# songrise/AvatarCraft

Hardware: AMD Instinct MI355X
Metric: rays/sec, 4096-ray batch, 256x256 render (64+64 samples/ray) (higher is better)
Workload: dtype f32

## Files before the change

### avatarcraft_amd/csrc/nsr_device.hpp

```cpp
#pragma once
#include "ac_common.hpp"
#include "ac_devmath.hpp"
#include "ac_sp_table.hpp"
#include "ac_sh16.hpp"

using namespace acdev;

typedef float f32x4 __attribute__((ext_vector_type(4)));

namespace {

#ifndef AC_WPB
#define AC_WPB 8
#endif
constexpr int WAVES_PER_BLOCK = AC_WPB;
constexpr int BLOCK = WAVES_PER_BLOCK * 64;
constexpr int MAXT = 128;
constexpr int SEG_STATE = MAXT + 16 + 64;
#ifndef AC_ENC_ROUND
#define AC_ENC_ROUND 2
#endif

constexpr int OFF_W1F = 0;
constexpr int OFF_W2F = OFF_W1F + 4 * 9 * 64;
// ... 7 lines not shown
constexpr int SPQ_FLOATS = 129 * 4;
constexpr int OFF_SPQ = OFF_LIN + 80;
constexpr int OFF_WAVE = OFF_SPQ + SPQ_FLOATS;
constexpr int FE_SLAB = 6 * 8 * 64;
constexpr int OFF_W1H = OFF_WAVE;
constexpr int OFF_W1L = OFF_W1H + 4 * 64 * 4;
constexpr int OFF_W1C = OFF_W1L + 4 * 64 * 4;
constexpr int CF_FRAGS = 14, CF_FRAG = 64 * 4;
constexpr int OFF_CFH = OFF_C1F;
constexpr int OFF_CFL = OFF_C1F + CF_FRAGS * CF_FRAG;
constexpr int OFF_C3L = OFF_W1C + 3 * 64;
static_assert(OFF_CFL + 12 * CF_FRAG == OFF_B1, "the bf16 colour fragments fill the fp32 colour region exactly");
constexpr int OFF_RWAVE = OFF_C3L + 2 * CF_FRAG;
constexpr int CF_OVERLAY = OFF_B1 - OFF_C1F;
constexpr int UPS_FLOATS = MAXT + 2 * MAXT + MAXT + 32;
constexpr int SLAB_ACC = MAXT + (FE_SLAB > UPS_FLOATS ? FE_SLAB : UPS_FLOATS);
constexpr int SLAB_SHB = SLAB_ACC + 16;
constexpr int WAVE_SLAB = SLAB_SHB + 80;
constexpr int LDS_FLOATS = OFF_RWAVE + WAVES_PER_BLOCK * WAVE_SLAB;
static_assert(LDS_FLOATS * 4 <= 160 * 1024, "LDS budget: one workgroup per CU");
static_assert(OFF_WAVE % 4 == 0 && OFF_RWAVE % 4 == 0 && WAVE_SLAB % 4 == 0, "16-byte aligned slabs");

#ifdef AC_PROFILE
#define AC_T0() unsigned long long t_prof_ = __builtin_amdgcn_s_memtime(); const unsigned long long ray_r0_ = __builtin_amdgcn_s_memrealtime()
#define AC_TICK(SLOT) { const unsigned long long t2_ = __builtin_amdgcn_s_memtime(); prof_acc[SLOT] += t2_ - t_prof_; t_prof_ = t2_; }
#else
#define AC_T0()
#define AC_TICK(SLOT)
#endif

struct LevelRec { float scale; uint32_t my, mz, offset, mask, hashed, wsize, pad; };

struct RenderArgs {
    const float *table;
    uint32_t table_bytes;
    const float *W1, *b1, *W2, *b2, *Wc1, *Wc2, *Wc3;
    const float *Wsh;
    const float *prepared;
    const float *rays_o, *rays_d, *bg, *noise, *lin_z, *lin_u;
    ac_render_out out;
    LevelRec lvl[16];
    int n_rays, T0, nup;
    int jmode[4];
    int jfine[4];
    float bound, two_bound, inv_s, car, one_m_car, eps;
    float inv_tb;
    const float *inv_s_dev;
    int fast;
    int skip_masked;
    int opacity_only;
    int perturb;
    unsigned long long *prof;
    const float *near_m, *far_m;
    const float *ext_pts;
    const uint8_t *mask;
    uint32_t *ray_counter;
    uint32_t *seg_flags;
    float *seg_state;
    uint64_t seg_cb;
    int seg_n;
    int pair_n;
    uint32_t *done_counter;
    uint32_t *handoff_timeouts;
    float *eik_red;
    uint32_t gen;
    int ex_from;
    int ex_rows;
    const uint8_t *ray_dead;
    float *zbuf;
    float *mid_pts;
};

enum { MODE_FULL = 0, MODE_UPSAMPLE = 2, MODE_FINAL = 3 };

__device__ __forceinline__ void cube_near_far(float ox, float oy, float oz, float dx, float dy, float dz, float bound, float &near, float &far)
{
    const float ex = dx + 1e-15f, ey = dy + 1e-15f, ez = dz + 1e-15f;
    const float ax = (-bound - ox) / ex, bx = (bound - ox) / ex;
    const float ay = (-bound - oy) / ey, by = (bound - oy) / ey;
    const float az = (-bound - oz) / ez, bz = (bound - oz) / ez;
    const float lx = ax < bx ? ax : bx, hx = ax > bx ? ax : bx;
    const float ly = ay < by ? ay : by, hy = ay > by ? ay : by;
    const float lz = az < bz ? az : bz, hz = az > bz ? az : bz;
    near = lx; if (ly > near) near = ly; if (lz > near) near = lz;
    far = hx; if (hy < far) far = hy; if (hz < far) far = hz;
    if (near < 0.05f) near = 0.05f;
}
__device__ __forceinline__ bool is_inf(float v) { return __builtin_fabsf(v) == __builtin_inff(); }

__device__ __forceinline__ void wave_sync()
{
    __builtin_amdgcn_fence(__ATOMIC_ACQ_REL, "wavefront");
    __builtin_amdgcn_wave_barrier();
}

template <int OFF> __device__ __forceinline__ float dpp_shr(float ident, float v)
{
    return __builtin_bit_cast(float, __builtin_amdgcn_update_dpp(__builtin_bit_cast(int, ident), __builtin_bit_cast(int, v),
                                                                  0x110 + OFF, 0xf, 0xf, false));
}
template <bool MUL> __device__ __forceinline__ float row_scan(float v)
{
    const float id = MUL ? 1.0f : 0.0f;
    float s;
    s = dpp_shr<1>(id, v); v = MUL ? s * v : s + v;
    s = dpp_shr<2>(id, v); v = MUL ? s * v : s + v;
    s = dpp_shr<4>(id, v); v = MUL ? s * v : s + v;
    s = dpp_shr<8>(id, v); v = MUL ? s * v : s + v;
    return v;
}
__device__ __forceinline__ float lane_bcast(float v, int lane)
{
    return __builtin_bit_cast(float, __builtin_amdgcn_readlane(__builtin_bit_cast(int, v), lane));
}
__device__ __forceinline__ float sel4(int g, float a, float b, float c, float d)
{
    return g == 0 ? a : (g == 1 ? b : (g == 2 ? c : d));
}

__device__ __forceinline__ void fill_lds_sdf(float *lds, const RenderArgs &a)
{
    for (int e = threadIdx.x; e < 4 * 9 * 64; e += blockDim.x) {
        int l = e & 63, fs = e >> 6, t = fs / 9, s = fs % 9;
        int u = 16 * t + (l & 15), g = l >> 4;
        int col = (s == 0) ? (g < 3 ? g : -1) : 3 + 2 * (4 * ((s - 1) >> 1) + g) + ((s - 1) & 1);
        lds[OFF_W1F + e] = col < 0 ? 0.0f : a.W1[u * 35 + col];
    }
    for (int e = threadIdx.x; e < 16 * 64; e += blockDim.x) {
        int l = e & 63, kk = e >> 6, t = kk >> 2, r = kk & 3;
        lds[OFF_W2F + e] = a.W2[(l & 15) * 64 + 16 * t + 4 * (l >> 4) + r];
    }
    for (int e = threadIdx.x; e < 64; e += blockDim.x) lds[OFF_B1 + e] = a.b1[e];
    for (int e = threadIdx.x; e < 16; e += blockDim.x) lds[OFF_B2 + e] = a.b2[e];
    {
        uint32_t *lw = reinterpret_cast<uint32_t *>(lds) + OFF_LVL;
#pragma unroll
        for (int l = 0; l < 16; ++l) {
            if (threadIdx.x == (unsigned)l) {
                lw[8 * l + 0] = __float_as_uint(a.lvl[l].scale); lw[8 * l + 1] = a.lvl[l].my;
                lw[8 * l + 2] = a.lvl[l].mz; lw[8 * l + 3] = a.lvl[l].offset;
                lw[8 * l + 4] = a.lvl[l].mask; lw[8 * l + 5] = a.lvl[l].hashed;
                lw[8 * l + 6] = a.lvl[l].wsize; lw[8 * l + 7] = 0u;
            }
        }
    }
    for (int e = threadIdx.x; e < 64; e += blockDim.x) lds[OFF_LIN + e] = e < a.T0 ? a.lin_z[e] : 0.0f;
    for (int e = threadIdx.x; e < 16; e += blockDim.x) lds[OFF_LIN + 64 + e] = a.lin_u ? a.lin_u[e] : 0.0f;
    for (int e = threadIdx.x; e < SPQ_FLOATS; e += blockDim.x) lds[OFF_SPQ + e] = AC_SP_G[e >> 2][e & 3];
}

__device__ __forceinline__ void fill_lds_color(float *lds, const RenderArgs &a)
{
    for (int e = threadIdx.x; e < 4 * 6 * 64; e += blockDim.x) {
        int l = e & 63, fs = e >> 6, t = fs / 6, s = fs % 6;
        int u = 16 * t + (l & 15), g = l >> 4;
        float v;
        if (s < 4) { int o = 4 * g + s; v = (o == 0) ? 0.0f : a.Wc1[u * 21 + 6 + (o - 1)]; }
        else if (s == 4) v = g < 3 ? a.Wc1[u * 21 + g] : 0.0f;
        else v = g < 3 ? a.Wc1[u * 21 + 3 + g] : 0.0f;
        lds[OFF_C1F + e] = v;
    }
    for (int e = threadIdx.x; e < 4 * 16 * 64; e += blockDim.x) {
        int l = e & 63, fs = e >> 6, to = fs >> 4, kk = fs & 15, t = kk >> 2, r = kk & 3;
        lds[OFF_C2F + e] = a.Wc2[(16 * to + (l & 15)) * 64 + 16 * t + 4 * (l >> 4) + r];
    }
    for (int e = threadIdx.x; e < 16 * 64; e += blockDim.x) {
        int l = e & 63, kk = e >> 6, t = kk >> 2, r = kk & 3, o = l & 15;
        lds[OFF_C3F + e] = o < 3 ? a.Wc3[o * 64 + 16 * t + 4 * (l >> 4) + r] : 0.0f;
    }
}

__device__ __forceinline__ void fill_lds(float *lds, const RenderArgs &a)
{
    fill_lds_sdf(lds, a);
    fill_lds_color(lds, a);
}

__device__ __forceinline__ uint32_t bf16_rne_bits(float f)
{
    const uint32_t u = __float_as_uint(f);
    return (u + 0x7fffu + ((u >> 16) & 1u)) >> 16;
}
template <int W1H = OFF_W1H, int W1L = OFF_W1L, int W1C = OFF_W1C>
__device__ __forceinline__ void fill_lds_fast(float *lds, const RenderArgs &a)
{
    uint32_t *lw = reinterpret_cast<uint32_t *>(lds);
    for (int e = threadIdx.x; e < 4 * 64 * 4; e += blockDim.x) {
        const int q = e & 3, l = (e >> 2) & 63, t = e >> 8;
        const int u = 16 * t + (l & 15), kk = l >> 4;
        uint32_t hi2 = 0, lo2 = 0;
#pragma unroll
        for (int h = 0; h < 2; ++h) {
            const int i = 2 * q + h;
            const float w = a.W1[u * 35 + 3 + 2 * (4 * (i >> 1) + kk) + (i & 1)];
            const uint32_t hb = bf16_rne_bits(w);
            const uint32_t lb = bf16_rne_bits(w - __uint_as_float(hb << 16));
            hi2 |= hb << (16 * h); lo2 |= lb << (16 * h);
        }
        lw[W1H + e] = hi2; lw[W1L + e] = lo2;
    }
    for (int e = threadIdx.x; e < 3 * 64; e += blockDim.x) lds[W1C + e] = a.W1[(e & 63) * 35 + (e >> 6)];
}

__device__ __forceinline__ float color_fast_weight(const RenderArgs &a, int f, int l, int i)
{
    const int m = l & 15, g = l >> 4;
    if (f < 4) {
        const int u = 16 * f + m;
        if (i < 4) { const int o = 4 * g + i; return o == 0 ? 0.0f : a.Wc1[u * 21 + 5 + o]; }
        if (i < 7 && g < 2) return a.Wc1[u * 21 + 3 * g + (i - 4)];
        return 0.0f;
    }
    const int s = (f - 4) & 1, unit = 16 * (2 * s + (i >> 2)) + 4 * g + (i & 3);
    if (f < 12) return a.Wc2[(16 * ((f - 4) >> 1) + m) * 64 + unit];
    return m < 3 ? a.Wc3[m * 64 + unit] : 0.0f;
}
template <bool OVERLAY, bool TAIL>
__device__ __forceinline__ void fill_lds_color_fast(float *lds, const RenderArgs &a)
{
    uint32_t *lw = reinterpret_cast<uint32_t *>(lds);
    for (int e = threadIdx.x; e < CF_FRAGS * CF_FRAG; e += blockDim.x) {
        const int q = e & 3, l = (e >> 2) & 63, f = e >> 8;
        if (!(f < 12 ? OVERLAY : (OVERLAY || TAIL))) continue;
        uint32_t hi2 = 0, lo2 = 0;
#pragma unroll
        for (int h = 0; h < 2; ++h) {
            const float w = color_fast_weight(a, f, l, 2 * q + h);
            const uint32_t hb = bf16_rne_bits(w);
            const uint32_t lb = bf16_rne_bits(w - __uint_as_float(hb << 16));
            hi2 |= hb << (16 * h); lo2 |= lb << (16 * h);
        }
        if (OVERLAY) lw[OFF_CFH + e] = hi2;
        if (f < 12) { if (OVERLAY) lw[OFF_CFL + e] = lo2; }
        else if (TAIL) lw[OFF_C3L + (e - 12 * CF_FRAG)] = lo2;
    }
}

typedef __amdgpu_buffer_rsrc_t rsrc_t;
typedef uint32_t u32x2 __attribute__((ext_vector_type(2)));
typedef uint32_t u32q __attribute__((ext_vector_type(4)));
__device__ __forceinline__ void interp8(const u32x2 (&v)[8], float qx, float qy, float qz, bool oob, float &f0, float &f1)
{
    const float wx0 = 1.0f - qx, wy0 = 1.0f - qy, wz0 = 1.0f - qz;
    const float w00 = wx0 * wy0, w10 = qx * wy0, w01 = wx0 * qy, w11 = qx * qy;
    float a0 = 0.0f, a1 = 0.0f;
#pragma unroll
    for (int c = 0; c < 8; ++c) {
        const float wxy = (c & 2) ? ((c & 1) ? w11 : w01) : ((c & 1) ? w10 : w00);
        const float w = wxy * ((c & 4) ? qz : wz0);
        a0 = fma_(w, __uint_as_float(v[c].x), a0);
        a1 = fma_(w, __uint_as_float(v[c].y), a1);
    }
    f0 = oob ? 0.0f : a0;
    f1 = oob ? 0.0f : a1;
}
template <int ROUND>
__device__ __forceinline__ void encode4(const float *__restrict__ lds, rsrc_t table, int g, const int (&jmode)[4],
                                        float px, float py, float pz, float bound, float two_bound, float (&f)[4][2], float inv_tb = 0.0f)
{
    float ux, uy, uz;
    if (inv_tb != 0.0f) { ux = unit_div(px + bound, two_bound, inv_tb); uy = unit_div(py + bound, two_bound, inv_tb); uz = unit_div(pz + bound, two_bound, inv_tb); }
    else { ux = (px + bound) / two_bound; uy = (py + bound) / two_bound; uz = (pz + bound) / two_bound; }
    const bool oob = (ux < 0.0f) | (ux > 1.0f) | (uy < 0.0f) | (uy > 1.0f) | (uz < 0.0f) | (uz > 1.0f);
#pragma unroll
    for (int j0 = 0; j0 < 4; j0 += ROUND) {
        float q[ROUND][3];
        u32x2 v[ROUND][8];
#pragma unroll
        for (int jj = 0; jj < ROUND; ++jj) {
            const int j = j0 + jj;
            const uint4 r0 = *reinterpret_cast<const uint4 *>(lds + OFF_LVL + (4 * j + g) * 8);
            const uint4 r1 = *reinterpret_cast<const uint4 *>(lds + OFF_LVL + (4 * j + g) * 8 + 4);
            const float scale = __uint_as_float(r0.x);
            const uint32_t my = r0.y, mz = r0.z, offset = r0.w, mask = r1.x, hashed = r1.y;
            float qx = fma_(ux, scale, 0.5f), qy = fma_(uy, scale, 0.5f), qz = fma_(uz, scale, 0.5f);
            const uint32_t gx = (uint32_t)__builtin_floorf(qx), gy = (uint32_t)__builtin_floorf(qy), gz = (uint32_t)__builtin_floorf(qz);
            q[jj][0] = qx - (float)gx; q[jj][1] = qy - (float)gy; q[jj][2] = qz - (float)gz;
            const uint32_t ax0 = gx, ax1 = gx + 1u, ay0 = gy * my, ay1 = ay0 + my, az0 = gz * mz, az1 = az0 + mz;
            const int mode = jmode[j];
            uint32_t idx[8];
            if (mode == 0) {
#pragma unroll
                for (int c = 0; c < 8; ++c) idx[c] = ((c & 1) ? ax1 : ax0) + ((c & 2) ? ay1 : ay0) + ((c & 4) ? az1 : az0);
            } else if (mode == 1) {
#pragma unroll
                for (int c = 0; c < 8; ++c) idx[c] = (((c & 1) ? ax1 : ax0) ^ ((c & 2) ? ay1 : ay0) ^ ((c & 4) ? az1 : az0)) & mask;
            } else {
#pragma unroll
                for (int c = 0; c < 8; ++c) {
                    const uint32_t tx = (c & 1) ? ax1 : ax0, ty = (c & 2) ? ay1 : ay0, tz = (c & 4) ? az1 : az0;
                    idx[c] = (hashed ? (tx ^ ty ^ tz) : (tx + ty + tz)) & mask;
                }
            }
#pragma unroll
            for (int c = 0; c < 8; ++c) v[jj][c] = __builtin_amdgcn_raw_buffer_load_b64(table, (offset + idx[c]) * 8u, 0, 0);
        }
#pragma unroll
        for (int jj = 0; jj < ROUND; ++jj)
            interp8(v[jj], q[jj][0], q[jj][1], q[jj][2], oob, f[j0 + jj][0], f[j0 + jj][1]);
        __builtin_amdgcn_sched_barrier(0);
    }
}

struct FieldCtx { rsrc_t table; int jmode[4]; int jfine[4]; float bound, two_bound, inv_tb; };
__device__ __forceinline__ rsrc_t table_of(const FieldCtx &fc) { return fc.table; }

struct Acc4 { f32x4 a[4]; };

__device__ __forceinline__ Acc4 sdf_l1(const float *__restrict__ lds, int lane, float bxyz, const float (&f)[4][2])
{
    const int g = lane >> 4;
    Acc4 acc;
#pragma unroll
    for (int t = 0; t < 4; ++t) acc.a[t] = *reinterpret_cast<const f32x4 *>(lds + OFF_B1 + 16 * t + 4 * g);
#pragma unroll
    for (int s = 0; s < 9; ++s) {
        const float b = (s == 0) ? bxyz : f[(s - 1) >> 1][(s - 1) & 1];
#pragma unroll
        for (int t = 0; t < 4; ++t)
            acc.a[t] = __builtin_amdgcn_mfma_f32_16x16x4f32(lds[OFF_W1F + (t * 9 + s) * 64 + lane], b, acc.a[t], 0, 0, 0);
    }
    return acc;
}

typedef __attribute__((ext_vector_type(8))) __bf16 bf16x8;
typedef uint32_t u32x4 __attribute__((ext_vector_type(4)));

__device__ __forceinline__ void split8_bf16(const float (&d)[8], u32x4 &bh, u32x4 &bl)
{
#pragma unroll
    for (int q = 0; q < 4; ++q) {
        const uint32_t u0 = __float_as_uint(d[2 * q]), u1 = __float_as_uint(d[2 * q + 1]);
        const float r0 = d[2 * q] - __uint_as_float(u0 & 0xffff0000u), r1 = d[2 * q + 1] - __uint_as_float(u1 & 0xffff0000u);
        bh[q] = __builtin_amdgcn_perm(u1, u0, 0x07060302u);
        bl[q] = __builtin_amdgcn_perm(__float_as_uint(r1), __float_as_uint(r0), 0x07060302u);
    }
}

template <int W1H = OFF_W1H, int W1L = OFF_W1L, int W1C = OFF_W1C>
__device__ __forceinline__ Acc4 sdf_l1_delta(const float *__restrict__ lds, int lane, const Acc4 &acc0, const float (&fe)[4][2],
                                             const float (&fe0)[4][2], int kn, float dcoord)
{
    const int g = lane >> 4;
    u32x4 bh, bl;
    float dlt[8];
#pragma unroll
    for (int q = 0; q < 4; ++q) { dlt[2 * q] = fe[q][0] - fe0[q][0]; dlt[2 * q + 1] = fe[q][1] - fe0[q][1]; }
    split8_bf16(dlt, bh, bl);
    const bf16x8 Bh = __builtin_bit_cast(bf16x8, bh), Bl = __builtin_bit_cast(bf16x8, bl);
    Acc4 r;
#pragma unroll
    for (int t = 0; t < 4; ++t) {
        const bf16x8 Ah = __builtin_bit_cast(bf16x8, *reinterpret_cast<const u32x4 *>(lds + W1H + (t * 64 + lane) * 4));
        const bf16x8 Al = __builtin_bit_cast(bf16x8, *reinterpret_cast<const u32x4 *>(lds + W1L + (t * 64 + lane) * 4));
        f32x4 c = __builtin_amdgcn_mfma_f32_16x16x32_bf16(Ah, Bh, acc0.a[t], 0, 0, 0);
        c = __builtin_amdgcn_mfma_f32_16x16x32_bf16(Al, Bh, c, 0, 0, 0);
        c = __builtin_amdgcn_mfma_f32_16x16x32_bf16(Ah, Bl, c, 0, 0, 0);
        const f32x4 wc = *reinterpret_cast<const f32x4 *>(lds + W1C + kn * 64 + 16 * t + 4 * g);
#pragma unroll
        for (int rr = 0; rr < 4; ++rr) c[rr] = fma_(dcoord, wc[rr], c[rr]);
        r.a[t] = c;
    }
    return r;
}

#ifndef AC_SP_BATCH
#define AC_SP_BATCH 4
#endif
__device__ __forceinline__ f32x4 sdf_l2(const float *__restrict__ lds, int lane, const Acc4 &acc)
{
    const int g = lane >> 4;
    f32x4 o2 = *reinterpret_cast<const f32x4 *>(lds + OFF_B2 + 4 * g);
#pragma unroll
    for (int t = 0; t < 4; ++t) {
        float h[4];
        const float xin[4] = { acc.a[t][0], acc.a[t][1], acc.a[t][2], acc.a[t][3] };
        dv_softplus100_n<4>(lds + OFF_SPQ, xin, h);
#pragma unroll
        for (int r = 0; r < 4; ++r)
            o2 = __builtin_amdgcn_mfma_f32_16x16x4f32(lds[OFF_W2F + (4 * t + r) * 64 + lane], h[r], o2, 0, 0, 0);
    }
    return o2;
}

struct W2Row0 { float w[4][4]; };
__device__ __forceinline__ W2Row0 load_w2_row0(const float *__restrict__ lds, int lane)
{
    W2Row0 r;
#pragma unroll
    for (int t = 0; t < 4; ++t)
#pragma unroll
        for (int q = 0; q < 4; ++q) r.w[t][q] = lds[OFF_W2F + (4 * t + q) * 64 + (lane & 48)];
    return r;
}
__device__ __forceinline__ float sdf_l2_sdf(const float *__restrict__ lds, const Acc4 &acc, const W2Row0 &w0)
{
    float p = 0.0f;
#pragma unroll
    for (int t0 = 0; t0 < 4; t0 += AC_SP_BATCH / 4) {
        constexpr int NB_ = AC_SP_BATCH;
        float xin[NB_], h[NB_];
#pragma unroll
        for (int i = 0; i < NB_; ++i) xin[i] = acc.a[t0 + (i >> 2)][i & 3];
        dv_softplus100_n<NB_>(lds + OFF_SPQ, xin, h);
#pragma unroll
        for (int i = 0; i < NB_; ++i) p = fma_(w0.w[t0 + (i >> 2)][i & 3], h[i], p);
    }
    const float other = __builtin_bit_cast(float, __builtin_amdgcn_ds_swizzle(__builtin_bit_cast(int, p), (0x10 << 10) | 0x1f));
    int lo = __builtin_bit_cast(int, p + other), hi = lo;
    asm volatile("s_nop 1\n\tv_permlane32_swap_b32 %0, %1" : "+v"(lo), "+v"(hi));
    return (__builtin_bit_cast(float, lo) + __builtin_bit_cast(float, hi)) + lds[OFF_B2];
}

__device__ __forceinline__ f32x4 sdf_mlp(const float *__restrict__ lds, int lane, float bxyz, const float (&f)[4][2])
{
    const Acc4 acc = sdf_l1(lds, lane, bxyz, f);
    __builtin_amdgcn_sched_barrier(0);
    return sdf_l2(lds, lane, acc);
}

__device__ __forceinline__ f32x4 sdf_tile(const float *__restrict__ lds, const FieldCtx &fc, int lane, float px, float py, float pz)
{
    const int g = lane >> 4;
    float f[4][2];
    encode4<AC_ENC_ROUND>(lds, fc.table, g, fc.jmode, px, py, pz, fc.bound, fc.two_bound, f, fc.inv_tb);
    __builtin_amdgcn_sched_barrier(0);
    return sdf_mlp(lds, lane, sel4(g, px, py, pz, 0.0f), f);
}

struct LvlC { float scale; uint32_t my, mz, offset, mask, hashed; };

template <int GM>
__device__ __forceinline__ uint32_t gidx(const LvlC &L, uint32_t tx, uint32_t ty, uint32_t tz)
{
    if constexpr (GM == 1) return (tx ^ ty ^ tz) & L.mask;
    else return (L.hashed ? (tx ^ ty ^ tz) : (tx + ty + tz)) & L.mask;
}
template <int K> __device__ __forceinline__ constexpr int face_corner(int b, int i)
{
    return K == 0 ? (b | (i << 1)) : (K == 1 ? ((i & 1) | (b << 1) | ((i >> 1) << 2)) : (i | (b << 2)));
}

template <int K, int SIGN>
struct AxisGeo { float qk; bool need, oob; };

template <int K, int SIGN, int GM>
__device__ __forceinline__ AxisGeo<K, SIGN> coarse_issue(rsrc_t table, const LvlC &L, const uint32_t (&gc)[3], const uint32_t (&tx)[2],
                                                       const uint32_t (&ty)[2], const uint32_t (&tz)[2], bool oob_c, float u,
                                                       u32x2 (&w)[4])
{
    AxisGeo<K, SIGN> a;
    a.oob = oob_c | (u < 0.0f) | (u > 1.0f);
    const float pos = fma_(u, L.scale, 0.5f);
    const uint32_t gk = (uint32_t)__builtin_floorf(pos);
    a.qk = pos - (float)gk;
    a.need = gk != gc[K];
    const uint32_t mk = K == 0 ? 1u : (K == 1 ? L.my : L.mz);
    const uint32_t base = K == 0 ? tx[0] : (K == 1 ? ty[0] : tz[0]);
    const uint32_t tk = SIGN == 0 ? base + 2u * mk : base - mk;
#pragma unroll
    for (int i = 0; i < 4; ++i) {
        const int c = face_corner<K>(0, i);
        const uint32_t ax = K == 0 ? tk : tx[c & 1], ay = K == 1 ? tk : ty[(c >> 1) & 1], az = K == 2 ? tk : tz[(c >> 2) & 1];
        w[i] = u32x2{ 0u, 0u };
        if (a.need) w[i] = __builtin_amdgcn_raw_buffer_load_b64(table, (L.offset + gidx<GM>(L, ax, ay, az)) * 8u, 0, 0);
    }
    return a;
}

template <int K, int SIGN>
__device__ __forceinline__ void coarse_finish(const AxisGeo<K, SIGN> &a, const u32x2 (&vc)[8], const u32x2 (&w)[4], const float (&qc)[3],
                                              float &f0, float &f1)
{
    constexpr int NEWBIT = SIGN == 0 ? 1 : 0;
    u32x2 v2[8];
#pragma unroll
    for (int c = 0; c < 8; ++c) {
        const int bk = (c >> K) & 1;
        const int i = K == 0 ? (c >> 1) : (K == 1 ? ((c & 1) | ((c >> 2) << 1)) : (c & 3));
        if (bk == NEWBIT) { v2[c].x = a.need ? w[i].x : vc[c].x; v2[c].y = a.need ? w[i].y : vc[c].y; }
        else { v2[c].x = a.need ? vc[c ^ (1 << K)].x : vc[c].x; v2[c].y = a.need ? vc[c ^ (1 << K)].y : vc[c].y; }
    }
    interp8(v2, K == 0 ? a.qk : qc[0], K == 1 ? a.qk : qc[1], K == 2 ? a.qk : qc[2], a.oob, f0, f1);
}


template <int K, int GM>
__device__ __forceinline__ void fine_issue(rsrc_t table, const LvlC &L, const uint32_t (&tx)[2], const uint32_t (&ty)[2],
                                           const uint32_t (&tz)[2], bool oob_c, float u, u32x2 (&v)[8], float &qk, bool &oob)
{
    oob = oob_c | (u < 0.0f) | (u > 1.0f);
    const float pos = fma_(u, L.scale, 0.5f);
    const uint32_t gk = (uint32_t)__builtin_floorf(pos);
    qk = pos - (float)gk;
    const uint32_t mk = K == 0 ? 1u : (K == 1 ? L.my : L.mz);
    const uint32_t t0 = gk * mk, t1 = t0 + mk;
#pragma unroll
    for (int c = 0; c < 8; ++c) {
        const uint32_t tk = ((c >> K) & 1) ? t1 : t0;
        const uint32_t ax = K == 0 ? tk : tx[c & 1], ay = K == 1 ? tk : ty[(c >> 1) & 1], az = K == 2 ? tk : tz[(c >> 2) & 1];
        v[c] = __builtin_amdgcn_raw_buffer_load_b64(table, (L.offset + gidx<GM>(L, ax, ay, az)) * 8u, 0, 0);
    }
}

#define AC_FSTORE(E, F0, F1) { fslab[((E - 1) * 8 + 2 * j) * 64 + lane] = F0; fslab[((E - 1) * 8 + 2 * j + 1) * 64 + lane] = F1; }

template <int GM>
__device__ __forceinline__ void stencil_levels(const float *__restrict__ lds, float *__restrict__ fslab, rsrc_t table, int lane, int g, int j, bool fine,
                                               float ux, float uy, float uz, bool oob, float xp, float xm, float yp, float ym, float zp, float zm,
                                               float &c0, float &c1)
{
    const uint4 r0 = *reinterpret_cast<const uint4 *>(lds + OFF_LVL + (4 * j + g) * 8);
    const uint4 r1 = *reinterpret_cast<const uint4 *>(lds + OFF_LVL + (4 * j + g) * 8 + 4);
    LvlC L; L.scale = __uint_as_float(r0.x); L.my = r0.y; L.mz = r0.z; L.offset = r0.w; L.mask = r1.x; L.hashed = r1.y;
    float qc[3]; uint32_t gc[3];
    {
        const float qx = fma_(ux, L.scale, 0.5f), qy = fma_(uy, L.scale, 0.5f), qz = fma_(uz, L.scale, 0.5f);
        gc[0] = (uint32_t)__builtin_floorf(qx); gc[1] = (uint32_t)__builtin_floorf(qy); gc[2] = (uint32_t)__builtin_floorf(qz);
        qc[0] = qx - (float)gc[0]; qc[1] = qy - (float)gc[1]; qc[2] = qz - (float)gc[2];
    }
    uint32_t tx[2], ty[2], tz[2];
    tx[0] = gc[0]; tx[1] = gc[0] + 1u; ty[0] = gc[1] * L.my; ty[1] = ty[0] + L.my; tz[0] = gc[2] * L.mz; tz[1] = tz[0] + L.mz;
    u32x2 vc[8];
#pragma unroll
    for (int c = 0; c < 8; ++c)
        vc[c] = __builtin_amdgcn_raw_buffer_load_b64(table, (L.offset + gidx<GM>(L, tx[c & 1], ty[(c >> 1) & 1], tz[c >> 2])) * 8u, 0, 0);
    if (!fine) {
        u32x2 w0[4], w1[4], w2[4], w3[4], w4[4], w5[4];
        const auto a0 = coarse_issue<0, 0, GM>(table, L, gc, tx, ty, tz, oob, xp, w0);
        const auto a1 = coarse_issue<0, 1, GM>(table, L, gc, tx, ty, tz, oob, xm, w1);
        const auto a2 = coarse_issue<1, 0, GM>(table, L, gc, tx, ty, tz, oob, yp, w2);
        const auto a3 = coarse_issue<1, 1, GM>(table, L, gc, tx, ty, tz, oob, ym, w3);
        const auto a4 = coarse_issue<2, 0, GM>(table, L, gc, tx, ty, tz, oob, zp, w4);
        const auto a5 = coarse_issue<2, 1, GM>(table, L, gc, tx, ty, tz, oob, zm, w5);
        __builtin_amdgcn_sched_barrier(0);
        interp8(vc, qc[0], qc[1], qc[2], oob, c0, c1);
        float f0, f1;
        coarse_finish<0, 0>(a0, vc, w0, qc, f0, f1); AC_FSTORE(1, f0, f1)
        coarse_finish<0, 1>(a1, vc, w1, qc, f0, f1); AC_FSTORE(2, f0, f1)
        coarse_finish<1, 0>(a2, vc, w2, qc, f0, f1); AC_FSTORE(3, f0, f1)
        coarse_finish<1, 1>(a3, vc, w3, qc, f0, f1); AC_FSTORE(4, f0, f1)
        coarse_finish<2, 0>(a4, vc, w4, qc, f0, f1); AC_FSTORE(5, f0, f1)
        coarse_finish<2, 1>(a5, vc, w5, qc, f0, f1); AC_FSTORE(6, f0, f1)
    } else {
        u32x2 va[8], vb[8], vc2[8], vd[8], ve[8], vf[8];
        float qa, qb, qc2, qd, qe, qf, f0, f1; bool oa, ob, oc2, od, oe, of;
        fine_issue<0, GM>(table, L, tx, ty, tz, oob, xp, va, qa, oa);
        fine_issue<0, GM>(table, L, tx, ty, tz, oob, xm, vb, qb, ob);
        fine_issue<1, GM>(table, L, tx, ty, tz, oob, yp, vc2, qc2, oc2);
        fine_issue<1, GM>(table, L, tx, ty, tz, oob, ym, vd, qd, od);
        fine_issue<2, GM>(table, L, tx, ty, tz, oob, zp, ve, qe, oe);
        fine_issue<2, GM>(table, L, tx, ty, tz, oob, zm, vf, qf, of);
        __builtin_amdgcn_sched_barrier(0);
        interp8(vc, qc[0], qc[1], qc[2], oob, c0, c1);
        interp8(va, qa, qc[1], qc[2], oa, f0, f1); AC_FSTORE(1, f0, f1)
        interp8(vb, qb, qc[1], qc[2], ob, f0, f1); AC_FSTORE(2, f0, f1)
        interp8(vc2, qc[0], qc2, qc[2], oc2, f0, f1); AC_FSTORE(3, f0, f1)
        interp8(vd, qc[0], qd, qc[2], od, f0, f1); AC_FSTORE(4, f0, f1)
        interp8(ve, qc[0], qc[1], qe, oe, f0, f1); AC_FSTORE(5, f0, f1)
        interp8(vf, qc[0], qc[1], qf, of, f0, f1); AC_FSTORE(6, f0, f1)
    }
}

__device__ __forceinline__ void encode_stencil(const float *__restrict__ lds, float *__restrict__ fslab, const FieldCtx &fc, int lane,
                                               float px, float py, float pz, float eps, float (&fe0)[4][2])
{
    const int g = lane >> 4;
    const rsrc_t table = fc.table;
    const float bound = fc.bound, two_bound = fc.two_bound, inv_tb = fc.inv_tb;
    const float ax = px + bound, ay = py + bound, az = pz + bound;
    const float axp = clampf(px + eps, -bound, bound) + bound, axm = clampf(px + (-eps), -bound, bound) + bound;
    const float ayp = clampf(py + eps, -bound, bound) + bound, aym = clampf(py + (-eps), -bound, bound) + bound;
    const float azp = clampf(pz + eps, -bound, bound) + bound, azm = clampf(pz + (-eps), -bound, bound) + bound;
    float ux, uy, uz, xp, xm, yp, ym, zp, zm;
    if (inv_tb != 0.0f) {
        ux = unit_div(ax, two_bound, inv_tb); uy = unit_div(ay, two_bound, inv_tb); uz = unit_div(az, two_bound, inv_tb);
        xp = unit_div(axp, two_bound, inv_tb); xm = unit_div(axm, two_bound, inv_tb); yp = unit_div(ayp, two_bound, inv_tb);
        ym = unit_div(aym, two_bound, inv_tb); zp = unit_div(azp, two_bound, inv_tb); zm = unit_div(azm, two_bound, inv_tb);
    } else {
        ux = ax / two_bound; uy = ay / two_bound; uz = az / two_bound;
        xp = axp / two_bound; xm = axm / two_bound; yp = ayp / two_bound; ym = aym / two_bound; zp = azp / two_bound; zm = azm / two_bound;
    }
    const bool oob = (ux < 0.0f) | (ux > 1.0f) | (uy < 0.0f) | (uy > 1.0f) | (uz < 0.0f) | (uz > 1.0f);
    const uint32_t jbits = (uint32_t)fc.jmode[0] | ((uint32_t)fc.jmode[1] << 2) | ((uint32_t)fc.jmode[2] << 4) | ((uint32_t)fc.jmode[3] << 6)
                         | ((fc.jfine[0] ? 1u : 0u) << 8) | ((fc.jfine[1] ? 1u : 0u) << 9) | ((fc.jfine[2] ? 1u : 0u) << 10) | ((fc.jfine[3] ? 1u : 0u) << 11);
#pragma unroll 1
    for (int j = 0; j < 4; ++j) {
        float c0, c1;
        const bool fine = (jbits >> (8 + j)) & 1u, hashed4 = ((jbits >> (2 * j)) & 3u) == 1u, dense4 = ((jbits >> (2 * j)) & 3u) == 0u;
        (void)dense4;
        if (hashed4) stencil_levels<1>(lds, fslab, table, lane, g, j, fine, ux, uy, uz, oob, xp, xm, yp, ym, zp, zm, c0, c1);
        else stencil_levels<2>(lds, fslab, table, lane, g, j, fine, ux, uy, uz, oob, xp, xm, yp, ym, zp, zm, c0, c1);
        fe0[0][0] = fe0[1][0]; fe0[0][1] = fe0[1][1]; fe0[1][0] = fe0[2][0]; fe0[1][1] = fe0[2][1];
        fe0[2][0] = fe0[3][0]; fe0[2][1] = fe0[3][1]; fe0[3][0] = c0; fe0[3][1] = c1;
        __builtin_amdgcn_sched_barrier(0);
    }
}
#undef AC_FSTORE

template <bool KEEP_SH = false>
__device__ __forceinline__ void ray_sh_bias(float *__restrict__ shb, const float *__restrict__ Wsh, float dx, float dy, float dz, int lane)
{
    float sh[16];
    ac_sh16(dx, dy, dz, sh);
    const f32x4 *w = reinterpret_cast<const f32x4 *>(Wsh + lane * 16);
    float acc = 0.0f;
// ... 203 lines not shown
```

### avatarcraft_amd/csrc/render_fused.hip

```cpp
#include <atomic>
#include <map>
#include <mutex>
#include "nsr_device.hpp"

namespace {

#ifndef AC_XCD_CHUNK
#define AC_XCD_CHUNK 512
#endif
template <int MODE, bool FAST, bool EX, bool SH = false>
__global__ __launch_bounds__(BLOCK) void render_rays_kernel(const RenderArgs a)
{
    constexpr bool FC = FAST;
    extern __shared__ __attribute__((aligned(16))) float lds[];
    if (a.prepared) {
        const float4 *src = reinterpret_cast<const float4 *>(a.prepared);
        float4 *dst = reinterpret_cast<float4 *>(lds);
        for (int e = threadIdx.x; e < OFF_RWAVE / 4; e += blockDim.x)
            dst[e] = src[(FC && 4 * e >= OFF_C1F && 4 * e < OFF_B1) ? e + (OFF_RWAVE - OFF_C1F) / 4 : e];
        __syncthreads();
        for (int e = threadIdx.x; e < 64; e += blockDim.x) lds[OFF_LIN + e] = e < a.T0 ? a.lin_z[e] : 0.0f;
        for (int e = threadIdx.x; e < 16; e += blockDim.x) lds[OFF_LIN + 64 + e] = a.lin_u ? a.lin_u[e] : 0.0f;
    } else {
        fill_lds_sdf(lds, a);
        if constexpr (FAST) fill_lds_fast(lds, a);
        if constexpr (FC) fill_lds_color_fast<true, true>(lds, a);
        else fill_lds_color(lds, a);
    }
    __syncthreads();

    const int lane = threadIdx.x & 63, wave = threadIdx.x >> 6;
    const int n = lane & 15, g = lane >> 4;
    float *zs0 = lds + OFF_RWAVE + wave * WAVE_SLAB;
    float *zs1 = zs0 + MAXT;
    float *sd = zs1 + MAXT;
    float *cdf = sd + 2 * MAXT;
    float *znl = cdf + MAXT;
    float *fsl = zs1;
    const FieldCtx fc = make_ctx(a);
    const W2Row0 w2r0 = load_w2_row0(lds, lane);
    const float bound = a.bound;
    const float inv_s_core = a.inv_s_dev ? *a.inv_s_dev : a.inv_s;
    const int T0 = a.T0, nup = a.nup, T = T0 + 16 * nup;

#ifdef AC_PROFILE
    unsigned long long prof_acc[8] = {0, 0, 0, 0, 0, 0, 0, 0};
    const unsigned long long prof_t0 = __builtin_amdgcn_s_memtime(), prof_r0 = __builtin_amdgcn_s_memrealtime();
#endif
    int bid = blockIdx.x;
    {
        const int k = blockIdx.x & 7, q = gridDim.x >> 3, r = gridDim.x & 7;
        bid = k * q + (k < r ? k : r) + (blockIdx.x >> 3);
    }
#ifndef AC_START_STAGGER
#define AC_START_STAGGER 1
#endif
    if (a.n_rays >= 2048)
        for (int k_ = 0; k_ < AC_START_STAGGER * wave; ++k_) __builtin_amdgcn_s_sleep(64);
    const int xper = ((a.n_rays + 7) / 8 + 7) & ~7, xchunk = xper < AC_XCD_CHUNK ? xper : AC_XCD_CHUNK, xcd = blockIdx.x & 7;
    const int seg_n = (MODE == MODE_UPSAMPLE) ? 1 : a.seg_n;
    for (int seg = 0; seg < seg_n; ++seg) {
    const int c_begin = (MODE == MODE_UPSAMPLE) ? 0 : (int)((a.seg_cb >> (4 * seg)) & 15u), c_end = (MODE == MODE_UPSAMPLE) ? 0 : (int)((a.seg_cb >> (4 * seg + 4)) & 15u);
    const bool seg_first = seg == 0, seg_last = seg + 1 == seg_n;
    for (;;) {
        int ray = 0;
        if (lane == 0) ray = (int)atomicAdd(a.ray_counter + xcd * 8 + seg, 1u);
        ray = __builtin_amdgcn_readfirstlane(ray);
        {
            const int k = ray / xchunk, base = (k * 8 + xcd) * xchunk;
            if (base >= a.n_rays) break;
            ray = base + (ray - k * xchunk);
            if (ray >= a.n_rays) continue;
        }
        int rin = ray;
        if (a.pair_n) { rin = ray >> 1; ray = rin + ((ray & 1) ? a.pair_n : 0); }
        (void)bid;
        const int exr = ray - a.ex_from;
        const bool ex_on = exr >= 0;
        AC_T0();
        const float ox = a.rays_o[3 * rin], oy = a.rays_o[3 * rin + 1], oz = a.rays_o[3 * rin + 2];
        const float dx = a.rays_d[3 * rin], dy = a.rays_d[3 * rin + 1], dz = a.rays_d[3 * rin + 2];
        float near, far;
        cube_near_far(ox, oy, oz, dx, dy, dz, bound, near, far);
        if (a.near_m) {
            const float nm = a.near_m[rin], fm = a.far_m[rin];
            if (!is_inf(nm)) near = nm;
            if (!is_inf(fm)) far = fm;
        }
        const float span = far - near;
        const float sample_dist = span / (float)T0;
        int cur = (MODE == MODE_FINAL) ? 0 : (nup & 1), cnt = T0;
        float *const zs_first = cur ? zs1 : zs0;

        if constexpr (MODE == MODE_UPSAMPLE) {
            if (a.ray_dead && a.ray_dead[ray]) {
                for (int i = lane; i < T; i += 64) {
                    const int ic = i < T0 ? i : T0 - 1;
                    float zi = near + span * lds[OFF_LIN + ic];
                    if (a.perturb) zi = zi + (a.noise[(size_t)ray * T0 + ic] - 0.5f) * sample_dist;
                    const size_t si = (size_t)ray * T + i;
                    a.zbuf[si] = zi;
                    if (a.mid_pts) { a.mid_pts[3 * si] = ox + dx * zi; a.mid_pts[3 * si + 1] = oy + dy * zi; a.mid_pts[3 * si + 2] = oz + dz * zi; }
                }
                wave_sync();
                continue;
            }
        }
        if constexpr (MODE == MODE_FINAL) {
            for (int i = lane; i < T; i += 64) zs0[i] = a.zbuf[(size_t)ray * T + i];
        } else if (seg_first) {
            for (int c = 0; c < T0 / 16; ++c) {
                const int i = 16 * c + n;
                float zi = near + span * lds[OFF_LIN + i];
                if (a.perturb) zi = zi + (a.noise[(size_t)ray * T0 + i] - 0.5f) * sample_dist;
                if (nup > 0) {
                    float px, py, pz;
                    if (MODE == MODE_UPSAMPLE && a.ext_pts) {
                        const float *e = a.ext_pts + ((size_t)ray * T0 + i) * 3;
                        px = clampf(e[0], -bound, bound); py = clampf(e[1], -bound, bound); pz = clampf(e[2], -bound, bound);
                    } else {
                        px = clampf(ox + dx * zi, -bound, bound); py = clampf(oy + dy * zi, -bound, bound);
                        pz = clampf(oz + dz * zi, -bound, bound);
                    }
                    const f32x4 o2 = sdf_tile(lds, fc, lane, px, py, pz);
                    if (g == 0) sd[cur * MAXT + i] = o2[0];
                }
                if (g == 0) zs_first[i] = zi;
            }
        }
        wave_sync();
        AC_TICK(0)

        for (int it = 0; it < ((MODE == MODE_FINAL || !seg_first) ? 0 : nup); ++it) {
            const float *zc = cur ? zs1 : zs0, *sc = sd + cur * MAXT;
            float *zn_ = cur ? zs0 : zs1, *sn_ = sd + (cur ^ 1) * MAXT;
            const int m = cnt - 1;
            const float inv_s = (float)(64 << it);
            float w[2];
            float carry = 1.0f; bool first = true;
#pragma unroll
            for (int ch = 0; ch < 2; ++ch) {
                const int i = 64 * ch + lane;
                float alpha = 0.0f, om = 1.0f;
                if (i < m) {
                    const float z0 = zc[i], z1 = zc[i + 1], s0 = sc[i], s1 = sc[i + 1];
                    const float p0x = ox + dx * z0, p0y = oy + dy * z0, p0z = oz + dz * z0;
                    const float p1x = ox + dx * z1, p1y = oy + dy * z1, p1z = oz + dz * z1;
                    const float r0 = __builtin_sqrtf((p0x * p0x + p0y * p0y) + p0z * p0z);
                    const float r1 = __builtin_sqrtf((p1x * p1x + p1y * p1y) + p1z * p1z);
                    const bool inside = (r0 < 1.0f) | (r1 < 1.0f);
                    const float mid = (s0 + s1) * 0.5f;
                    const float dist = z1 - z0;
                    const float cosv = (s1 - s0) / (dist + 1e-5f);
                    float prev_cos = 0.0f;
                    if (i > 0) { const float zm = zc[i - 1], sm = sc[i - 1]; prev_cos = (s0 - sm) / ((z0 - zm) + 1e-5f); }
                    float cmin = prev_cos < cosv ? prev_cos : cosv;
                    cmin = clampf(cmin, -1e3f, 0.0f) * (inside ? 1.0f : 0.0f);
                    const float half = cmin * dist * 0.5f;
                    const float pc = dv_sigmoid((mid - half) * inv_s), nc = dv_sigmoid((mid + half) * inv_s);
                    alpha = (pc - nc + 1e-5f) / (pc + 1e-5f);
                    om = 1.0f - alpha + 1e-7f;
                }
                float loc, row_in; bool row_first;
                (void)chunk_scan<true>(om, lane, carry, first, loc, row_in, row_first);
                const float sh = dpp_shr<1>(1.0f, loc);
                float Tex;
                if (n == 0) Tex = row_first ? 1.0f : row_in;
                else Tex = row_first ? sh : row_in * sh;
                w[ch] = (i < m) ? alpha * Tex + 1e-5f : 0.0f;
            }
            float total;
            {
                float c2 = 0.0f; bool f2 = true; float lc, ri; bool rf;
                float last = 0.0f;
#pragma unroll
                for (int ch = 0; ch < 2; ++ch) {
                    const float incl = chunk_scan<false>(w[ch], lane, c2, f2, lc, ri, rf);
                    const int il = m - 1 - 64 * ch;
                    const float cand = __shfl(incl, il & 63);
                    if (il >= 0 && il < 64) last = cand;
                }
                total = last;
            }
            {
                float c3 = 0.0f; bool f3 = true; float lc, ri; bool rf;
                if (lane == 0) cdf[0] = 0.0f;
#pragma unroll
                for (int ch = 0; ch < 2; ++ch) {
                    const int i = 64 * ch + lane;
                    const float pdf = (i < m) ? w[ch] / total : 0.0f;
                    const float incl = chunk_scan<false>(pdf, lane, c3, f3, lc, ri, rf);
                    if (i < m) cdf[i + 1] = incl;
                }
            }
            wave_sync();
            float znew;
            int ind;
            {
                const float u = lds[OFF_LIN + 64 + n];
                int lo = 0, hi = cnt;
                while (lo < hi) { const int md = (lo + hi) >> 1; if (cdf[md] <= u) lo = md + 1; else hi = md; }
                ind = lo;
                const int below = lo - 1 > 0 ? lo - 1 : 0;
                const int above = lo < cnt - 1 ? lo : cnt - 1;
                const float cb = cdf[below], ca = cdf[above];
                float den = ca - cb;
                if (den < 1e-5f) den = 1.0f;
                const float t = (u - cb) / den;
                const float zb = zc[below], za = zc[above];
                znew = zb + t * (za - zb);
            }
            if (g == 0) {
                znl[n] = znew;
                if (EX && ex_on && a.out.ss_inds) a.out.ss_inds[((size_t)exr * nup + it) * 16 + n] = ind;
            }
            AC_TICK(1)
            const bool last_it = (it + 1 == nup);
            float sdf_new = 0.0f;
            if (!last_it) {
                const float px = clampf(ox + dx * znew, -bound, bound), py = clampf(oy + dy * znew, -bound, bound),
                            pz = clampf(oz + dz * znew, -bound, bound);
                const f32x4 o2 = sdf_tile(lds, fc, lane, px, py, pz);
                sdf_new = o2[0];
            }
            wave_sync();
            AC_TICK(2)
            const bool old_sorted = !(it == 0 && span < 0.0f);
            int32_t *sidx = (EX && ex_on && a.out.sort_index) ? a.out.sort_index + ((size_t)exr * nup + it) * 128 : nullptr;
#pragma unroll
            for (int ch = 0; ch < 2; ++ch) {
                const int i = 64 * ch + lane;
                if (i < cnt) {
                    const float zi = zc[i];
                    int c = 0;
#pragma unroll
                    for (int j = 0; j < 16; ++j) c += (znl[j] < zi) ? 1 : 0;
                    int before = i;
                    if (!old_sorted) {
                        before = 0;
                        for (int k = 0; k < cnt; ++k) { const float zk = zc[k]; before += ((zk < zi) || (zk == zi && k < i)) ? 1 : 0; }
                    }
                    zn_[before + c] = zi; sn_[before + c] = sc[i];
                    if (sidx) sidx[before + c] = i;
                }
                if (sidx && i >= cnt + 16) sidx[i] = -1;
            }
            if (g == 0) {
                int lo = 0, hi = cnt;
                if (old_sorted) {
                    while (lo < hi) { const int md = (lo + hi) >> 1; if (zc[md] <= znew) lo = md + 1; else hi = md; }
                } else {
                    for (int k = 0; k < cnt; ++k) lo += (zc[k] <= znew) ? 1 : 0;
                }
                int c = 0;
#pragma unroll
                for (int j = 0; j < 16; ++j) { const float zj = znl[j]; c += ((zj < znew) || (zj == znew && j < n)) ? 1 : 0; }
                zn_[lo + c] = znew; sn_[lo + c] = sdf_new;
                if (sidx) sidx[lo + c] = cnt + n;
            }
            cnt += 16; cur ^= 1;
            wave_sync();
            AC_TICK(1)
        }

        const float *zf = zs0;
        if constexpr (MODE == MODE_UPSAMPLE) {
            for (int i = lane; i < T; i += 64) {
                const float zi = zf[i];
                const float delta = (i < T - 1) ? zf[i + 1] - zi : sample_dist;
                const float zmid = (i < T - 1) ? zi + 0.5f * delta : zi;
                const size_t si = (size_t)ray * T + i;
                a.zbuf[si] = zi;
                if (a.mid_pts) { a.mid_pts[3 * si] = ox + dx * zmid; a.mid_pts[3 * si + 1] = oy + dy * zmid; a.mid_pts[3 * si + 2] = oz + dz * zmid; }
            }
            wave_sync();
            continue;
        }
        float cT = 1.0f;
        float *const accs = zs0 + SLAB_ACC;
        if constexpr (SH && MODE != MODE_UPSAMPLE) { if (seg_first && !a.opacity_only) ray_sh_bias(zs0 + SLAB_SHB, a.Wsh, dx, dy, dz, lane); }
        if (!seg_first) {
            int timed_out = 0;
            if (lane == 0) {
                int spins = 0;
                for (;;) {
                    const uint32_t f = __hip_atomic_load(a.seg_flags + ray, __ATOMIC_RELAXED, __HIP_MEMORY_SCOPE_AGENT);
                    if (((f >> 4) == a.gen && (f & 15u) >= (uint32_t)seg) || spins >= (1 << 21)) break;
                    __builtin_amdgcn_s_sleep(8); ++spins;
                }
                timed_out = spins >= (1 << 21);
                if (timed_out && a.handoff_timeouts) atomicAdd(a.handoff_timeouts, 1u);
            }
            timed_out = __builtin_amdgcn_readfirstlane(timed_out);
            wave_sync();
            const uint32_t *st = reinterpret_cast<const uint32_t *>(a.seg_state + (size_t)ray * SEG_STATE);
            if constexpr (MODE != MODE_FINAL)
                for (int i = lane; i < T; i += 64) zs0[i] = __uint_as_float(__hip_atomic_load(st + i, __ATOMIC_RELAXED, __HIP_MEMORY_SCOPE_AGENT));
            const float cv = __uint_as_float(__hip_atomic_load(st + MAXT + (lane & 15), __ATOMIC_RELAXED, __HIP_MEMORY_SCOPE_AGENT));
            cT = lane_bcast(cv, 0);
            if (lane < 16) accs[lane] = cv;
            if constexpr (SH) zs0[SLAB_SHB + lane] = __uint_as_float(__hip_atomic_load(st + MAXT + 16 + lane, __ATOMIC_RELAXED, __HIP_MEMORY_SCOPE_AGENT));
            if (timed_out) {
                cT = __builtin_nanf("");
                if (lane < 16) accs[lane] = cT;
            }
            wave_sync();
        }
        const float bxe = a.eps;
        const int c_hi = c_end < T / 16 ? c_end : T / 16;
        for (int c = c_begin; c < c_hi; ++c) {
            const int i = 16 * c + n;
            const float zi = zf[i];
            const float delta = (i < T - 1) ? zf[i + 1] - zi : sample_dist;
            const float zmid = (i < T - 1) ? zi + 0.5f * delta : zi;
            float px, py, pz;
            if constexpr (MODE == MODE_FINAL) {
                const float *e = a.ext_pts + ((size_t)ray * T + i) * 3;
                px = clampf(e[0], -bound, bound); py = clampf(e[1], -bound, bound); pz = clampf(e[2], -bound, bound);
            } else {
                px = clampf(ox + dx * zmid, -bound, bound); py = clampf(oy + dy * zmid, -bound, bound);
                pz = clampf(oz + dz * zmid, -bound, bound);
            }
            AC_TICK(7)
            bool skip = false;
            if constexpr (MODE == MODE_FINAL) {
                if (a.skip_masked) skip = __ballot(a.mask[(size_t)ray * T + i] != 0) == 0ull;
            }
            f32x4 oc = { 0.0f, 0.0f, 0.0f, 0.0f };
            float gr[3] = { 0.0f, 0.0f, 0.0f };
            if (!skip) {
            float fe0[4][2];
            encode_stencil(lds, fsl, fc, lane, px, py, pz, bxe, fe0);
            if (EX && ex_on && a.out.feat7) {
                int lane_x = lane;
                asm volatile("" : "+v"(lane_x));
                f32x4 *dst = reinterpret_cast<f32x4 *>(a.out.feat7) + (((size_t)exr * (T / 16) + (i >> 4)) * 14) * 64 + lane_x;
                dst[0] = f32x4{ fe0[0][0], fe0[0][1], fe0[1][0], fe0[1][1] };
                dst[64] = f32x4{ fe0[2][0], fe0[2][1], fe0[3][0], fe0[3][1] };
#pragma unroll 1
                for (int e = 0; e < 6; ++e) {
                    const float *sp = fsl + (e * 8) * 64 + lane;
                    dst[(2 * e + 2) * 64] = f32x4{ sp[0], sp[64], sp[128], sp[192] };
                    dst[(2 * e + 3) * 64] = f32x4{ sp[256], sp[320], sp[384], sp[448] };
                }
            }
            AC_TICK(3)
            const float pc0 = sel4(g, px, py, pz, 0.0f);
            float spos = 0.0f;
            if constexpr (FAST) {
                const Acc4 acc0 = sdf_l1(lds, lane, pc0, fe0);
                oc = sdf_l2(lds, lane, acc0);
#pragma unroll 1
                for (int e = 0; e < 6; ++e) {
                    const int kn = e >> 1;
                    float fe[4][2];
#pragma unroll
                    for (int q_ = 0; q_ < 8; ++q_) fe[q_ >> 1][q_ & 1] = fsl[(e * 8 + q_) * 64 + lane];
                    const float pk = kn == 0 ? px : (kn == 1 ? py : pz);
                    const float poff = clampf(pk + ((e & 1) ? -bxe : bxe), -bound, bound);
                    const Acc4 acc = sdf_l1_delta(lds, lane, acc0, fe, fe0, kn, poff - pk);
                    const float s_e = sdf_l2_sdf(lds, acc, w2r0);
                    if (!(e & 1)) spos = s_e;
                    else {
                        const float gk = 0.5f * (spos - s_e) / bxe;
                        if (kn == 0) gr[0] = gk; else if (kn == 1) gr[1] = gk; else gr[2] = gk;
                    }
                }
            } else {
            Acc4 acc = sdf_l1(lds, lane, pc0, fe0);
#pragma unroll 1
            for (int e = 0; e < 7; ++e) {
                Acc4 accn = acc;
                if (e < 6) {
                    const int kn = e >> 1;
                    float fe[4][2];
#pragma unroll
                    for (int q_ = 0; q_ < 8; ++q_) fe[q_ >> 1][q_ & 1] = fsl[(e * 8 + q_) * 64 + lane];
                    const float pk = kn == 0 ? px : (kn == 1 ? py : pz);
                    const float poff = clampf(pk + ((e & 1) ? -bxe : bxe), -bound, bound);
                    accn = sdf_l1(lds, lane, g == kn ? poff : pc0, fe);
                }
                if (e == 0) oc = sdf_l2(lds, lane, acc);
                else {
                    const float s_e = sdf_l2_sdf(lds, acc, w2r0);
                    const int k = (e - 1) >> 1;
                    if (e & 1) spos = s_e;
                    else {
                        const float gk = 0.5f * (spos - s_e) / bxe;
                        if (k == 0) gr[0] = gk; else if (k == 1) gr[1] = gk; else gr[2] = gk;
                    }
                }
                acc = accn;
            }
            }
            }
            AC_TICK(4)
            const float gx = gr[0], gy = gr[1], gz = gr[2];
            const float gn = __builtin_sqrtf((gx * gx + gy * gy) + gz * gz);
            const float nx = gx / (1e-5f + gn), ny = gy / (1e-5f + gn), nz = gz / (1e-5f + gn);
            float rgb[3] = { 0.0f, 0.0f, 0.0f };
            if (!skip && !a.opacity_only) {
                if constexpr (FC) color_tile_fast(lds, lane, px, py, pz, nx, ny, nz, oc, rgb, nullptr, 16, SH ? zs0 + SLAB_SHB : nullptr);
                else color_tile(lds, lane, px, py, pz, nx, ny, nz, oc, rgb, nullptr, 16, SH ? zs0 + SLAB_SHB : nullptr);
            }
            AC_TICK(5)
            const float sdf0 = oc[0];
            const float tc = (dx * nx + dy * ny) + dz * nz;
            const float a1 = dv_softplus100(lds + OFF_SPQ, -tc * 0.5f + 0.5f) * a.one_m_car;
            const float a2 = dv_softplus100(lds + OFF_SPQ, -tc) * a.car;
            const float iter_cos = -(a1 + a2);
            const float half = iter_cos * delta * 0.5f;
            const float pc = dv_sigmoid((sdf0 - half) * inv_s_core), nc = dv_sigmoid((sdf0 + half) * inv_s_core);
            float alpha = clampf((pc - nc + 1e-5f) / (pc + 1e-5f), 0.0f, 1.0f);
            if constexpr (MODE == MODE_FINAL) alpha = alpha * (a.mask[(size_t)ray * T + i] ? 1.0f : 0.0f);
            const float om = 1.0f - alpha + 1e-7f;
            const float loc = row_scan<true>(om);
            const float sh = dpp_shr<1>(1.0f, loc);
            float Tex;
            if (n == 0) Tex = (c == 0) ? 1.0f : cT;
            else Tex = (c == 0) ? sh : cT * sh;
            const float tot = lane_bcast(loc, 15);
            cT = (c == 0) ? tot : cT * tot;
            const float wgt = alpha * Tex;
            const float zn01 = clampf((zi - near) / span, 0.0f, 1.0f);
            const float pn = __builtin_sqrtf((px * px + py * py) + pz * pz);
            const float relax = (pn < 1.2f && !skip) ? 1.0f : 0.0f;
            const float eerr = relax * ((gn - 1.0f) * (gn - 1.0f));
            {
                const float t1 = row_scan<false>(wgt), t2 = row_scan<false>(rgb[0] * wgt), t3 = row_scan<false>(rgb[1] * wgt), t4 = row_scan<false>(rgb[2] * wgt),
                            t5 = row_scan<false>(nx * wgt), t6 = row_scan<false>(ny * wgt), t7 = row_scan<false>(nz * wgt), t8 = row_scan<false>(wgt * zn01),
// ... 586 lines not shown
```

Baseline: 5.430 million.

## Software-pipeline coarse SDF hash-grid gathers with the MLP of the previous tile

```diff
diff --git a/avatarcraft_amd/csrc/nsr_device.hpp b/avatarcraft_amd/csrc/nsr_device.hpp
--- a/avatarcraft_amd/csrc/nsr_device.hpp
+++ b/avatarcraft_amd/csrc/nsr_device.hpp
@@ -333,6 +333,51 @@
     }
 }
 
+struct Gath4 { u32x2 v[4][8]; float q[4][3]; bool oob; };
+__device__ __forceinline__ Gath4 encode4_issue(const float *__restrict__ lds, rsrc_t table, int g, const int (&jmode)[4],
+                                               float px, float py, float pz, float bound, float two_bound, float inv_tb)
+{
+    Gath4 r;
+    float ux, uy, uz;
+    if (inv_tb != 0.0f) { ux = unit_div(px + bound, two_bound, inv_tb); uy = unit_div(py + bound, two_bound, inv_tb); uz = unit_div(pz + bound, two_bound, inv_tb); }
+    else { ux = (px + bound) / two_bound; uy = (py + bound) / two_bound; uz = (pz + bound) / two_bound; }
+    r.oob = (ux < 0.0f) | (ux > 1.0f) | (uy < 0.0f) | (uy > 1.0f) | (uz < 0.0f) | (uz > 1.0f);
+#pragma unroll
+    for (int j = 0; j < 4; ++j) {
+        const uint4 r0 = *reinterpret_cast<const uint4 *>(lds + OFF_LVL + (4 * j + g) * 8);
+        const uint4 r1 = *reinterpret_cast<const uint4 *>(lds + OFF_LVL + (4 * j + g) * 8 + 4);
+        const float scale = __uint_as_float(r0.x);
+        const uint32_t my = r0.y, mz = r0.z, offset = r0.w, mask = r1.x, hashed = r1.y;
+        const float qx = fma_(ux, scale, 0.5f), qy = fma_(uy, scale, 0.5f), qz = fma_(uz, scale, 0.5f);
+        const uint32_t gx = (uint32_t)__builtin_floorf(qx), gy = (uint32_t)__builtin_floorf(qy), gz = (uint32_t)__builtin_floorf(qz);
+        r.q[j][0] = qx - (float)gx; r.q[j][1] = qy - (float)gy; r.q[j][2] = qz - (float)gz;
+        const uint32_t ax0 = gx, ax1 = gx + 1u, ay0 = gy * my, ay1 = ay0 + my, az0 = gz * mz, az1 = az0 + mz;
+        const int mode = jmode[j];
+        uint32_t idx[8];
+        if (mode == 0) {
+#pragma unroll
+            for (int c = 0; c < 8; ++c) idx[c] = ((c & 1) ? ax1 : ax0) + ((c & 2) ? ay1 : ay0) + ((c & 4) ? az1 : az0);
+        } else if (mode == 1) {
+#pragma unroll
+            for (int c = 0; c < 8; ++c) idx[c] = (((c & 1) ? ax1 : ax0) ^ ((c & 2) ? ay1 : ay0) ^ ((c & 4) ? az1 : az0)) & mask;
+        } else {
+#pragma unroll
+            for (int c = 0; c < 8; ++c) {
+                const uint32_t tx = (c & 1) ? ax1 : ax0, ty = (c & 2) ? ay1 : ay0, tz = (c & 4) ? az1 : az0;
+                idx[c] = (hashed ? (tx ^ ty ^ tz) : (tx + ty + tz)) & mask;
+            }
+        }
+#pragma unroll
+        for (int c = 0; c < 8; ++c) r.v[j][c] = __builtin_amdgcn_raw_buffer_load_b64(table, (offset + idx[c]) * 8u, 0, 0);
+    }
+    return r;
+}
+__device__ __forceinline__ void encode4_finish(const Gath4 &r, float (&f)[4][2])
+{
+#pragma unroll
+    for (int j = 0; j < 4; ++j) interp8(r.v[j], r.q[j][0], r.q[j][1], r.q[j][2], r.oob, f[j][0], f[j][1]);
+}
+
 struct FieldCtx { rsrc_t table; int jmode[4]; int jfine[4]; float bound, two_bound, inv_tb; };
 __device__ __forceinline__ rsrc_t table_of(const FieldCtx &fc) { return fc.table; }
 
diff --git a/avatarcraft_amd/csrc/render_fused.hip b/avatarcraft_amd/csrc/render_fused.hip
--- a/avatarcraft_amd/csrc/render_fused.hip
+++ b/avatarcraft_amd/csrc/render_fused.hip
@@ -109,23 +109,41 @@
         if constexpr (MODE == MODE_FINAL) {
             for (int i = lane; i < T; i += 64) zs0[i] = a.zbuf[(size_t)ray * T + i];
         } else if (seg_first) {
-            for (int c = 0; c < T0 / 16; ++c) {
-                const int i = 16 * c + n;
-                float zi = near + span * lds[OFF_LIN + i];
+            auto coarse_issue = [&](int i, float &zi, Gath4 &gv) -> float {
+                zi = near + span * lds[OFF_LIN + i];
                 if (a.perturb) zi = zi + (a.noise[(size_t)ray * T0 + i] - 0.5f) * sample_dist;
-                if (nup > 0) {
-                    float px, py, pz;
-                    if (MODE == MODE_UPSAMPLE && a.ext_pts) {
-                        const float *e = a.ext_pts + ((size_t)ray * T0 + i) * 3;
-                        px = clampf(e[0], -bound, bound); py = clampf(e[1], -bound, bound); pz = clampf(e[2], -bound, bound);
-                    } else {
-                        px = clampf(ox + dx * zi, -bound, bound); py = clampf(oy + dy * zi, -bound, bound);
-                        pz = clampf(oz + dz * zi, -bound, bound);
-                    }
-                    const f32x4 o2 = sdf_tile(lds, fc, lane, px, py, pz);
-                    if (g == 0) sd[cur * MAXT + i] = o2[0];
-                }
-                if (g == 0) zs_first[i] = zi;
+                float px, py, pz;
+                if (MODE == MODE_UPSAMPLE && a.ext_pts) {
+                    const float *e = a.ext_pts + ((size_t)ray * T0 + i) * 3;
+                    px = clampf(e[0], -bound, bound); py = clampf(e[1], -bound, bound); pz = clampf(e[2], -bound, bound);
+                } else {
+                    px = clampf(ox + dx * zi, -bound, bound); py = clampf(oy + dy * zi, -bound, bound);
+                    pz = clampf(oz + dz * zi, -bound, bound);
+                }
+                gv = encode4_issue(lds, fc.table, g, fc.jmode, px, py, pz, fc.bound, fc.two_bound, fc.inv_tb);
+                return sel4(g, px, py, pz, 0.0f);
+            };
+            if (nup > 0) {
+                float zi, f[4][2];
+                Gath4 gv;
+                float bx = coarse_issue(n, zi, gv);
+                for (int c = 0; c < T0 / 16; ++c) {
+                    const int i = 16 * c + n;
+                    encode4_finish(gv, f);
+                    const float zc = zi, bc = bx;
+                    __builtin_amdgcn_sched_barrier(0);
+                    if (c + 1 < T0 / 16) bx = coarse_issue(i + 16, zi, gv);
+                    __builtin_amdgcn_sched_barrier(0);
+                    const f32x4 o2 = sdf_mlp(lds, lane, bc, f);
+                    if (g == 0) { sd[cur * MAXT + i] = o2[0]; zs_first[i] = zc; }
+                }
+            } else {
+                for (int c = 0; c < T0 / 16; ++c) {
+                    const int i = 16 * c + n;
+                    float zi = near + span * lds[OFF_LIN + i];
+                    if (a.perturb) zi = zi + (a.noise[(size_t)ray * T0 + i] - 0.5f) * sample_dist;
+                    if (g == 0) zs_first[i] = zi;
+                }
             }
         }
         wave_sync();
```

Result: no change. 5.450 million, median of 6 (+0.4%).
